# wilsonCernWq/qaray

Hardware: AMD Instinct MI355X
Metric: Msamples/s (1 sample = 1 camera path), Cornell box 1080p@512spp (higher is better)
Workload: dtype f32

## Files before the change

include/qaray_hip.h:

```cpp
#ifndef QARAY_HIP_H
#define QARAY_HIP_H

#include <stdint.h>

#include "qa_flat_scene.h"
#include "qa_photon.h"
#include "qaray_host.h"

#ifdef __cplusplus
extern "C" {
#endif

typedef struct qa_ctx qa_ctx;

typedef struct qa_counters {
  uint64_t samples;
  uint64_t casts_normal;
  uint64_t casts_shadow;
  uint64_t bvh_nodes;
  uint64_t tri_tests;
  uint64_t pixels;
} qa_counters;

#define QA_RENDER_STATS 1u
// ... 17 lines not shown
int qa_scene_edit_texels(qa_ctx *ctx, uint32_t texture, int x0, int y0, int x1, int y1, const uint8_t *rgb8, uint64_t row_stride_bytes);
int qa_scene_edit_texels_device(qa_ctx *ctx, uint32_t texture, int x0, int y0, int x1, int y1, const uint8_t *d_rgb8,
                                uint64_t row_stride_bytes, void *hip_stream);

int qa_render_region(qa_ctx *ctx, int x0, int y0, int x1, int y1, int spp_min, int spp_max,
                     int max_bounce, uint32_t seed, uint32_t flags, float *rgb, float *depth,
                     uint32_t *nsamples);
int qa_render_region_device(qa_ctx *ctx, int x0, int y0, int x1, int y1, int spp_min, int spp_max,
                            int max_bounce, uint32_t seed, uint32_t flags, float *d_rgb,
                            float *d_depth, uint32_t *d_nsamples, void *hip_stream);
#define QA_STRIP_ROWS 8
int qa_render_strips_device(qa_ctx *ctx, int x0, int y0, int x1, int y1, int first_strip, int strip_step,
                            int spp_min, int spp_max, int max_bounce, uint32_t seed, uint32_t flags,
                            float *d_rgb, float *d_depth, uint32_t *d_nsamples, void *hip_stream);
int qa_strip_count(int y0, int y1, int first_strip, int strip_step);
int qa_synchronize(qa_ctx *ctx);

int qa_photon_maps_build(qa_ctx *ctx, const qa_photon_params *params, uint32_t seed);
int qa_photon_maps_clear(qa_ctx *ctx);
int qa_photon_maps_info(qa_ctx *ctx, uint64_t emitted[2], uint64_t emissions[2]);
int qa_photon_maps_download(qa_ctx *ctx, int which, qa_photon *out, uint64_t capacity);

int qa_request_stop(qa_ctx *ctx);
int qa_clear_stop(qa_ctx *ctx);

int qa_progressive_begin(qa_ctx *ctx, int x0, int y0, int x1, int y1, int spp_min, int spp_max, int max_bounce, uint32_t seed,
                         uint32_t flags);
int qa_progressive_advance(qa_ctx *ctx, int spp_target, void *hip_stream);
int qa_progressive_read(qa_ctx *ctx, float *rgb, float *depth, uint32_t *nsamples);
int qa_progressive_read_device(qa_ctx *ctx, float *d_rgb, float *d_depth, uint32_t *d_nsamples, void *hip_stream);
// ... 200 lines not shown
```

qaray_amd/csrc/hip/qa_capi.hip:

```cpp
#include <hip/hip_runtime.h>

#include <algorithm>
#include <cstddef>
#include <cstring>
#include <new>

#include "qa_ctx.h"
#include "qa_radiance.h"
#include "qa_ray_query.h"

static int EnsurePlanSlab(qa_ctx *c)
{
  const size_t threads = (size_t) c->numCUs * 8 * QA_BLOCK;
  const bool area = c->plan.area, many = !area && c->plan.shadowLights.size() > QA_CS_LIGHT_BATCH;
  float **slab = area ? &c->dAreaSlab : many ? &c->dSurfSlab : nullptr;
  if (slab && !*slab) {
    void *p = nullptr;
    HIP_TRY(hipMalloc(&p, threads * (area ? kAreaLogFloats : 13) * sizeof(float)));
    c->sceneAllocs.push_back(p);
    c->statSceneAllocs++;
    *slab = static_cast<float *>(p);
  }
  c->ds.areaScratch = area ? c->dAreaSlab : nullptr;
  c->ds.csSurf = many ? c->dSurfSlab : nullptr;
// ... 391 lines not shown
  out->samples = h.samples;
  out->casts_normal = h.casts_normal;
  out->casts_shadow = h.casts_shadow;
  out->bvh_nodes = h.bvh_nodes;
  out->tri_tests = h.tri_tests;
  out->pixels = h.pixels;
#ifdef QA_STAMPS
  {
    const double w = (double) std::max<unsigned long long>(h.stamp[9], 1), k = (double) std::max<unsigned long long>(h.stamp[0], 1);
    fprintf(stderr, "[stamps] waves %llu, iterations/wave %.0f, cycles/wave %.3e | share of wave time: fetch+start %.3f, closest %.3f (mesh walks %.3f), shade %.3f, "
            "direct light %.3f (shadow mesh walks %.3f), sample end %.3f, miss branch %.3f, hit before shading %.3f, spawn %.3f\n", h.stamp[9], h.stamp[8] / w, k / w, h.stamp[1] / k, h.stamp[2] / k, h.stamp[3] / k,
            h.stamp[4] / k, h.stamp[5] / k, h.stamp[6] / k, h.stamp[7] / k, h.stamp[10] / k, h.stamp[11] / k, h.stamp[12] / k);
    if (h.stamp[19] || h.stamp[21])
      fprintf(stderr, "[stamps] waves without a camera ray: mesh walks of their closest-hit sweeps %.3f (the camera rays': %.3f), after the sweep %.3f | last-cast queries %.3f (mesh walks %.3f), %llu lanes asked again (of %llu casts)\n",
              h.stamp[19] / k, (h.stamp[3] - (double) h.stamp[19]) / k, h.stamp[20] / k, h.stamp[21] / k, h.stamp[22] / k, h.stamp[23], (unsigned long long) h.casts_normal);
    if (c->integ[kCs].fn && h.stamp[11])
      fprintf(stderr, "[stamps] cooperative walks: %llu rounds, %.1f of 64 lanes hold an item on average (lane occupancy of the walks %.3f); %.3f of the rounds are leaf rounds; 'mesh walks' above = the rounds alone\n", h.stamp[11],
              (double) h.stamp[10] / (double) h.stamp[11], (double) h.stamp[10] / (64.0 * (double) h.stamp[11]), (double) h.stamp[12] / (double) h.stamp[11]);
    if (c->integ[kCs].fn)
      fprintf(stderr, "[stamps] closest-hit sweeps without their rounds %.3f, winners' details %.3f, shadow sweeps without their rounds %.3f; lanes sent to the exact walks: %llu closest, %llu shadow (of %llu + %llu casts)\n",
              (h.stamp[13] - (double) h.stamp[3]) / k, h.stamp[14] / k, (h.stamp[17] - (double) h.stamp[6]) / k, h.stamp[15], h.stamp[16], (unsigned long long) h.casts_normal, (unsigned long long) h.casts_shadow);
  }
#endif
  return QA_OK;
}
int qa_reset_counters(qa_ctx *c)
{
  if (!c) return Fail(QA_EINVAL, "null context");
  if (int rc = qa_synchronize(c)) return rc;
  HIP_TRY(hipMemset(c->dCounters, 0, sizeof(DCounters)));
// ... 50 lines not shown
  return QA_OK;
}

int qa_set_option(qa_ctx *c, const char *name, long long value)
{
  if (!c || !name) return Fail(QA_EINVAL, "null argument");
  const std::string n(name);
  if (n == "coop") {
    c->optCoop = value != 0;
    if (c->haveScene) return SelectKernel(c);
  } else if (n == "cs_cull") c->optCsCull = value != 0;
  else if (n == "cs_force_exact") c->optCsForceExact = (uint32_t) (value & 3);
  else if (n == "walk_zero_terms") c->optWalkZeroTerms = value ? 1u : 0u;
  else if (n == "last_cast") c->optLastCast = value < 0 ? -1 : (value ? 1 : 0);
  else if (n == "leaf_sweep") c->optLeafSweep = value < 0 ? -1 : (value ? 1 : 0);
  else if (n == "chunk_spp") c->optChunkSpp = value < 0 ? -1 : (int) (value > 65535 ? 65535 : value);
  else if (n == "chunk_tail") c->optChunkTail = value < 0 ? 0 : (int) (value > 65535 ? 65535 : value);
  else if (n == "tile_lists") c->optTileLists = value < 0 ? -1 : (int) (value > QA_TILE_LEAF_CAP ? QA_TILE_LEAF_CAP : value);
  else if (n == "cs_pool_limit") c->optCsPool = value > 0 ? (uint32_t) std::max<long long>(64, value) : 0u;
  else if (n == "sync_samples") c->syncSamples = value < 0 ? -1 : (value > 64 ? 64 : (int) value);
  else if (n == "tile_order") c->tileOrder = value != 0;
  else if (n == "progressive_tile_limit") c->optProgTileLimit = value > 0 ? (uint32_t) std::min<long long>(value, 0x7FFFFFFF) : 0u;
  else if (n == "staged_groups") {
    c->wf.numGroups = (int) std::max<long long>(1, std::min<long long>(value, WfHost::kMaxGroups));
    if (c->haveScene) SetKernelName(c);
  } else if (n == "verbose") c->optVerbose = value != 0;
  else return Fail(QA_EINVAL, "unknown option '" + n + "'");
  return QA_OK;
}

// ... 11 lines not shown
```

qaray_amd/csrc/hip/qa_ctx.h:

```cpp
#pragma once
#include <hip/hip_runtime.h>

#include <cstdint>
#include <string>
#include <vector>

#include "qa_scene_build.h"
#include "qa_wf_types.h"
#include "qaray_hip.h"

using namespace qa;

typedef void (*KernelFn)(const DScene, const RenderParams);
KernelFn PickKernel(bool resident, bool lights, bool tex, bool area, bool stats);
KernelFn PickLastCastKernel();
KernelFn PickCs(bool lights, bool tex, bool cull, bool many, bool area);
KernelFn PickCsResume(bool lights, bool cull, bool many, bool area);
extern const int kMaxPath;
extern const size_t kAreaLogFloats;
size_t CsLdsBytes(uint32_t items, uint32_t slots);

inline thread_local std::string g_err;
inline int Fail(int code, const std::string &msg) { g_err = msg; return code; }
#define HIP_TRY(expr)                                                                          \
  do {                                                                                         \
    hipError_t e_ = (expr);                                                                    \
    if (e_ != hipSuccess) return Fail(QA_EHIP, std::string(#expr) + ": " + hipGetErrorString(e_)); \
  } while (0)

inline const char *DevEnv(const char *name)
// ... 135 lines not shown
  int syncSamples = -1;
  bool photonReady = false;
  void *dPhotons[2] = {nullptr, nullptr};
  void *dPmTables[2][3] = {{nullptr, nullptr, nullptr}, {nullptr, nullptr, nullptr}};
  void *dHeap = nullptr;
  qa_photon_params photonParams{};
  uint64_t photonEmitted[2] = {0, 0}, photonEmissions[2] = {0, 0};
  std::vector<qa_photon> hostPhotons[2];
  WfHost wf;
  std::string kernelName;
  std::string launchedName;
  bool optCoop = true;
  bool optCsCull = true;
  int optLastCast = -1;
  int optLeafSweep = -1;
  uint32_t optWalkZeroTerms = 0;
  uint32_t optCsForceExact = 0;
  uint32_t optCsPool = 0;
  bool optVerbose = false;
  uint32_t optProgTileLimit = 0;
  struct Progressive {
    bool active = false;
    bool stale = false;
    std::string ended;
    FrameArgs args;
    unsigned tiles = 0;
    size_t npix = 0;
    int target = 0;
    int top = 0;
    uint32_t *dState = nullptr;
// ... 103 lines not shown
```

qaray_amd/csrc/hip/qa_frame.hip:

```cpp
#include <algorithm>
#include <cstring>

#include "qa_ctx.h"

int EnsureHalton(qa_ctx *c, int count)
{
  if (count > c->haltonCount) {
    int n = 64;
    while (n < count) n *= 2;
    std::vector<float> t(2 * (size_t) n);
    for (int s = 0; s < n; ++s) { t[2 * s] = HaltonF(s, 11); t[2 * s + 1] = HaltonF(s, 13); }
    if (c->dHalton) (void) hipFree(c->dHalton);
    c->dHalton = nullptr;
    HIP_TRY(hipMalloc((void **) &c->dHalton, t.size() * sizeof(float)));
    HIP_TRY(hipMemcpy(c->dHalton, t.data(), t.size() * sizeof(float), hipMemcpyHostToDevice));
    c->haltonCount = n;
  }
  c->ds.halton = c->dHalton;
  c->ds.halton_count = c->haltonCount;
  return QA_OK;
}

static bool CsManyVariant(const qa_ctx *c) { return c->plan.shadowLights.size() > QA_CS_LIGHT_BATCH && !c->plan.area; }
static bool LastCastVariant(const qa_ctx *c) { return c->plan.resident && c->plan.lastCastQuery && c->ds.num_lights == 0; }
static bool CsCullVariant(const qa_ctx *c) { return c->plan.csCullOk && (CsManyVariant(c) || c->plan.area || c->plan.textured || c->ds.num_inst > 12); }

static std::string IntegratorName(const qa_ctx *c, Slot s)
{
  const ScenePlan &p = c->plan;
  const int lights = c->ds.num_lights > 0;
  char name[160];
  if (s == kCs || s == kCsResume)
    snprintf(name, sizeof(name), "qa_integrate_cs%s<LIGHTS=%d,TEX=%d,CULL=%d%s%s>", s == kCsResume ? "_resume" : "", lights, (int) p.textured, (int) CsCullVariant(c),
             CsManyVariant(c) ? ",MANY=1" : "", p.area ? ",AREA=1" : "");
  else snprintf(name, sizeof(name), "qa_integrate<RES=%d,LIGHTS=%d,TEX=%d,AREA=%d%s>", (int) p.resident, lights, (int) p.textured, (int) p.area,
                s == kMega && LastCastVariant(c) ? ",LASTCAST=1" : "");
  std::string out = name;
  if (s == kPm || s == kPmStats) out += " + photon-map gathers (PHOTON=1)";
  if (s == kMegaStats || s == kPmStats) out += " counting variant (STATS=1, reference tree)";
// ... 57 lines not shown
  return QA_OK;
}

int LaunchSetup(qa_ctx *c, Launch &L, const FrameArgs &a, int ownRows, unsigned int *work, bool resume)
{
  const hipStream_t s = a.stream;
  const int x0 = a.x0, y0 = a.y0, x1 = a.x1, y1 = a.y1;
  HIP_TRY(c->lastFrame.WaitOn(s));
  HIP_TRY(c->lastEdit.WaitOn(s));

  RenderParams &rp = L.rp;
  rp.x0 = x0; rp.y0 = y0; rp.x1 = x1; rp.y1 = y1;
  rp.spp_min = a.sppMin; rp.spp_max = a.sppMax; rp.max_bounce = a.maxBounce;
  rp.seed = a.seed;
  rp.tile_row0 = a.tileRow0; rp.tile_row_step = a.tileRowStep; rp.own_tile_rows = ownRows;
  rp.tile_lists = c->plan.tileListBytes ? (c->optTileLists < 0 ? QA_TILE_LISTS_AUTO : c->optTileLists) : 0;
  rp.sync_samples = c->syncSamples < 0 ? c->plan.syncAuto : c->syncSamples;
  rp.rgb = a.rgb; rp.depth = a.depth; rp.ns = a.ns;
  rp.work_counter = work;
  rp.tile_order = nullptr;
  {
    const int tx = (x1 - x0 + 7) / 8;
    const uint64_t key = ((uint64_t) tx << 40) ^ ((uint64_t) ownRows << 20) ^ ((uint64_t) a.tileRow0 << 8) ^ (uint64_t) a.tileRowStep ^
                         ((uint64_t) (y1 - y0) << 50);
    if (key != c->orderKey || !c->dOrder) {
      const size_t n = (size_t) tx * ownRows;
      std::vector<std::pair<float, uint32_t>> v(n);
      const float cx = 0.5f * (x1 - x0), cy = 0.5f * (y1 - y0);
      for (int r = 0; r < ownRows; ++r)
        for (int i = 0; i < tx; ++i) {
          const float px = i * 8 + 4 - cx, py = (a.tileRow0 + r * a.tileRowStep) * 8 + 4 - cy;
// ... 35 lines not shown
  if (cs && c->syncSamples < 0 && ((c->plan.syncAuto && c->plan.textured) || CsManyVariant(c))) rp.sync_samples = 32;
  if (cs && c->plan.area) rp.sync_samples = 1;
  ds.csCullOn = (c->optCsCull && c->plan.csCullOk) ? 1u : 0u;
  ds.csForceExact = c->optCsForceExact;
  ds.walkZeroTerms = c->optWalkZeroTerms;
  ds.lastCast = (LastCastVariant(c) && c->optLastCast != 0) ? (c->optLeafSweep != 0 ? 2u : 1u) : 0u;
  ds.lastCastGlow = c->plan.lastCastGlow;
  ds.csPoolLimit = DevEnv("QA_CS_POOL") ? (uint32_t) std::max(64, atoi(DevEnv("QA_CS_POOL"))) : c->optCsPool;

  L.tiles = (unsigned) ((x1 - x0 + 7) / 8) * (unsigned) ownRows;
  const long long needBlocks = ((long long) L.tiles * 64 + QA_BLOCK - 1) / QA_BLOCK;
  L.blocks = (long long) c->numCUs * (c->optBlocksPerCU > 0 ? c->optBlocksPerCU : c->integ[L.slot].blocksPerCU);
  if (pmOn && L.blocks > (long long) c->numCUs * 8) L.blocks = (long long) c->numCUs * 8;
  if (L.blocks > needBlocks) L.blocks = needBlocks;
  if (L.blocks < 1) L.blocks = 1;
  rp.chunk_spp = 0; rp.chunk_tail = 0; rp.num_chunks = 1; rp.chunk_pad = 0; rp.tile_progress = nullptr; rp.pix_state = nullptr;
  return QA_OK;
}

int LaunchFrame(qa_ctx *c, Launch &L, bool staged, hipStream_t s)
{
  EventPair ev;
  if (!c->freeEvents.empty()) { ev = c->freeEvents.back(); c->freeEvents.pop_back(); }
  else { HIP_TRY(hipEventCreate(&ev.a)); HIP_TRY(hipEventCreate(&ev.b)); }
  HIP_TRY(hipEventRecord(ev.a, s));
  if (staged) {
    const int rc = RenderStaged(c, L.ds, L.rp, s, L.rp.counters);
    if (rc != QA_OK) { c->freeEvents.push_back(ev); return rc; }
  } else {
    hipLaunchKernelGGL(c->integ[L.slot].fn, dim3((unsigned) L.blocks), dim3(QA_BLOCK), (unsigned) c->integ[L.slot].ldsBytes, s, L.ds, L.rp);
    HIP_TRY(hipGetLastError());
// ... 66 lines not shown
extern "C" {

int qa_render_region_device(qa_ctx *c, int x0, int y0, int x1, int y1, int spp_min, int spp_max, int max_bounce,
                            uint32_t seed, uint32_t flags, float *d_rgb, float *d_depth, uint32_t *d_ns, void *hip_stream)
{
  if (int rc = Enter(c)) return rc;
  return Render(c, {x0, y0, x1, y1, 0, 1, spp_min, spp_max, max_bounce, seed, flags, d_rgb, d_depth, d_ns, StreamOf(c, hip_stream)});
}

int qa_render_strips_device(qa_ctx *c, int x0, int y0, int x1, int y1, int first_strip, int strip_step, int spp_min,
                            int spp_max, int max_bounce, uint32_t seed, uint32_t flags, float *d_rgb, float *d_depth,
                            uint32_t *d_ns, void *hip_stream)
{
  if (int rc = Enter(c)) return rc;
  return Render(c, {x0, y0, x1, y1, first_strip, strip_step, spp_min, spp_max, max_bounce, seed, flags, d_rgb, d_depth, d_ns, StreamOf(c, hip_stream)});
}

int qa_strip_count(int y0, int y1, int first_strip, int strip_step)
{
  if (y1 <= y0 || first_strip < 0 || strip_step < 1) return 0;
  return OwnTileRows(y0, y1, first_strip, strip_step);
}

int qa_render_region(qa_ctx *c, int x0, int y0, int x1, int y1, int spp_min, int spp_max, int max_bounce,
                     uint32_t seed, uint32_t flags, float *rgb, float *depth, uint32_t *ns)
{
  if (!c || !rgb || !depth || !ns) return Fail(QA_EINVAL, "null argument");
  if (x1 <= x0 || y1 <= y0) return Fail(QA_EINVAL, "empty region");
  HIP_TRY(hipSetDevice(c->device));
  const size_t npix = (size_t) (x1 - x0) * (y1 - y0);
// ... 16 lines not shown
```

qaray_amd/csrc/hip/qa_kernel.h:

```cpp
#pragma once
#include <hip/hip_runtime.h>

#include <type_traits>

#include "qa_device_math.h"
#include "qa_scene_dev.h"
#include "qa_seed.h"
#include "qa_texture_dev.h"
#include "qa_tilecull.h"

namespace qa {

#ifndef QA_MIN_WAVES
#define QA_MIN_WAVES 4
#endif
#define QA_BIAS 0.005f
#define QA_DX 0.01f
#ifdef QA_WAVE_TALLIES
#define QA_TALLY(x) (x) += (unsigned long long) __popcll(__ballot(1))
#else
#define QA_LANE_TALLIES 1
#define QA_TALLY(x) (x)++
#endif

// ... 1353 lines not shown
    const uint32_t count = (uint32_t) __popcll(mask);
    if (count > limit || cursor + count > QA_TILE_LIST_CAP) continue;
    uint32_t rank = 0;
    for (unsigned long long rest = mask; rest; rest &= rest - 1) {
      const int j = __ffsll((long long) rest) - 1;
      const float bj = __shfl(bound, j);
      rank += (bj < bound || (bj == bound && j < (int) lane)) ? 1u : 0u;
    }
    if (cand) tl[QA_TILE_LIST_HDR + cursor + rank] = QA_TILE_ENTRY(word, __float_as_uint(bound));
    if (lane == 0) tl[mySlot] = 0x80000000u | (count << 8) | cursor;
    cursor += count;
  }
  __builtin_amdgcn_wave_barrier();
}

struct Path {
  Ray ray;
  f3 T;
  f3 L;
  int absorbMtl;
  int bounce;
  bool fromDiffuse;
  bool primary;
};

#define QA_MAX_PATH 8
#define QA_REC_FLOATS 19

#ifndef QA_C2_EXTRA_WAVE
#define QA_C2_EXTRA_WAVE 1
// ... 41 lines not shown
```

qaray_amd/csrc/hip/qa_kernel_lastcast_body.h:

```cpp
  extern __shared__ uint4 s_dyn[];
  SceneMem<RES> mem;
  mem.img = s_dyn;
  static_assert(RES, "the last-cast query belongs to the resident variant without lights");
  for (uint32_t i = threadIdx.x; i < sc.residentVec4; i += QA_BLOCK) s_dyn[i] = sc.resident[i];
  __syncthreads();
  uint32_t *stack = reinterpret_cast<uint32_t *>(s_dyn + sc.residentVec4) + threadIdx.x;
  float *acc = reinterpret_cast<float *>(stack + (size_t) sc.stackDepth * QA_BLOCK - threadIdx.x) + threadIdx.x;
  const uint4 *mtlTable = s_dyn + sc.resMaterials;
  for (int i = 12; i < QA_LANE_SLOTS_RES; ++i) acc[i * QA_BLOCK] = 0.f;
  constexpr bool TL = true;
  uint32_t *tileList = nullptr;
  if (rp.tile_lists > 0 && !(sc.cam.dof > 0.1f))
    tileList = reinterpret_cast<uint32_t *>(s_dyn + sc.residentVec4) + ((size_t) sc.stackDepth + QA_LANE_SLOTS_RES) * QA_BLOCK +
               __builtin_amdgcn_readfirstlane(threadIdx.x / 64) * QA_TILE_LIST_DWORDS;

  const int rw = rp.x1 - rp.x0, rh = rp.y1 - rp.y0;
  const unsigned tilesX = (unsigned) (rw + 7) / 8;
  const unsigned numTiles = tilesX * (unsigned) rp.own_tile_rows;
  const unsigned total = numTiles * (rp.chunk_spp ? rp.num_chunks : 1u) * 64u;
  const unsigned lane = __lane_id();
  unsigned curTile = 0xFFFFFFFFu, curChunk = 0;
  int chunkEnd = 0x7FFFFFFF;

  DCounters cnt = {};
// ... 3 lines not shown
  if (__lane_id() < QA_NSTAMPS) cnt.sl[__lane_id()] = 0;
#endif
  QA_T(tKernel)
  TexTables tt;
  tt.blob = sc.blob;
  tt.texels = sc.texels;
  tt.texOff = sc.texOff;
  tt.texmap = sc.texmap;
  tt.tex = sc.tex;
  tt.filter = sc.texFilter;
  RayDiff pathDiff;
  pathDiff.dx = pathDiff.dy = F3(0, 0, 1);

  uint32_t rng = 1;
  bool alive = true, needPixel = true;

  for (;;) {
    QA_T(tA)
    const unsigned long long aliveMask = __ballot(alive);
    const unsigned long long want = __ballot(alive && needPixel);
    if (want && want == aliveMask) {
      if (rp.chunk_spp && curTile != 0xFFFFFFFFu) {
        asm volatile("s_waitcnt vmcnt(0)" ::: "memory");
        if (lane == 0) __hip_atomic_store(rp.tile_progress + curTile, curChunk + 1u, __ATOMIC_RELAXED, __HIP_MEMORY_SCOPE_AGENT);
        curTile = 0xFFFFFFFFu;
      }
      unsigned base = 0;
      const int leader = __ffsll((long long) want) - 1;
      if ((int) lane == leader) base = (*rp.stop_flag) ? total : atomicAdd(rp.work_counter, 64u);
      base = __shfl(base, leader);
      unsigned item = base / 64;
      if (rp.chunk_spp && base < total) {
        curChunk = item / numTiles;
        item -= curChunk * numTiles;
        curTile = item;
        chunkEnd = (int) (rp.chunk_spp + curChunk * rp.chunk_tail);
        if (curChunk > 0) {
          for (int spins = 0; spins < (1 << 22); ++spins) {
            if (__hip_atomic_load(rp.tile_progress + curTile, __ATOMIC_RELAXED, __HIP_MEMORY_SCOPE_AGENT) >= curChunk) break;
            __builtin_amdgcn_s_sleep(16);
          }
          __builtin_amdgcn_fence(__ATOMIC_ACQUIRE, "agent");
        }
      }
      if (tileList && base < total) {
        const unsigned tile = rp.tile_order ? rp.tile_order[item] : item;
        const unsigned otr = tile / tilesX;
        buildTileLists<RES>(sc, (uint32_t) rp.tile_lists, (float) (rp.x0 + (int) ((tile % tilesX) * 8)),
                            (float) (rp.y0 + (int) (((unsigned) rp.tile_row0 + otr * (unsigned) rp.tile_row_step) * 8)), tileList,
                            reinterpret_cast<TileCone *>(stack - lane));
        rng = 1;
// ... 213 lines not shown
#undef QA_PAIR
          needPixel = true;
        }
      } else {
        rp.rgb[3 * qo + 0] = mean.x;
        rp.rgb[3 * qo + 1] = mean.y;
        rp.rgb[3 * qo + 2] = mean.z;
        rp.ns[qo] = (uint32_t) sidx;
        if (rp.chunk_spp)
          __hip_atomic_store(reinterpret_cast<unsigned long long *>(rp.pix_state) + 4 * (size_t) qo, 0x80000000ull << 32, __ATOMIC_RELAXED, __HIP_MEMORY_SCOPE_AGENT);
        QA_TALLY(cnt.pixels);
        needPixel = true;
      }
    }
    QA_TACC(cnt.sl[7], tE)
  }

  unsigned long long v[6] = {cnt.samples, cnt.casts_normal, cnt.casts_shadow, cnt.bvh_nodes, cnt.tri_tests, cnt.pixels};
  unsigned long long *dst = reinterpret_cast<unsigned long long *>(rp.counters);
  for (int i = 0; i < 6; ++i) {
    unsigned long long x = v[i];
#ifdef QA_LANE_TALLIES
    for (int off = 32; off > 0; off >>= 1) x += __shfl_down(x, off);
#endif
    if (lane == 0 && x) atomicAdd(&dst[i], x);
  }
#ifdef QA_STAMPS
  if (lane == 0) {
    cnt.sl[0] = __builtin_readcyclecounter() - tKernel;
    cnt.sl[9] = 1;
    for (int i = 0; i < QA_NSTAMPS; ++i) atomicAdd(&dst[6 + i], cnt.sl[i]);
// ... 3 lines not shown
```

qaray_amd/csrc/hip/qa_lastcast.hip:

```cpp
#include "qa_kernel.h"
#include "qa_ctx.h"

KernelFn PickLastCastKernel() { return (KernelFn) qa::qa_integrate_lastcast<true>; }
```

qaray_amd/csrc/hip/qa_probes.hip:

```cpp
#include <cstring>

#include "qa_device_math.h"
#include "qa_texture_dev.h"
#include "qa_ctx.h"

namespace qa {
__global__ __launch_bounds__(256, 8) void qa_scrub_scratch(uint32_t pattern, uint32_t *never)
{
  volatile uint32_t a[512];
  for (int i = 0; i < 512; ++i) a[i] = pattern;
  for (int i = 0; i < 300; ++i) __builtin_amdgcn_s_sleep(127);
  if (a[threadIdx.x] == 0x12345u && pattern != 0x12345u) never[0] = 1;
}
}

__global__ void qa_sincos_probe(const float *x, int n, float *s, float *c)
{
  const int i = blockIdx.x * blockDim.x + threadIdx.x;
  if (i < n) { s[i] = qsinf(x[i]); c[i] = qcosf(x[i]); }
}

__global__ void qa_math_probe(int fn, const float *x, const float *y, int n, float *out)
{
  const int i = blockIdx.x * blockDim.x + threadIdx.x;
// ... 166 lines not shown
  int mesh = 0, elem = 0;
  if (!TexProbeArgsOk(h, t.plan, op, index, n, &mesh, &elem)) return QA_EINVAL;
  TexTables tt;
  tt.blob = static_cast<const unsigned char *>(blob);
  tt.texels = reinterpret_cast<const float4 *>(t.texels.data());
  tt.texOff = t.texOff.data();
  tt.texmap = QA_BLOB_PTR(qa_texmap, blob, h->off_texmaps);
  tt.tex = QA_BLOB_PTR(qa_texture, blob, h->off_textures);
  tt.filter = t.taps.data();
  const DTri *tris = op == 8 ? t.mesh[mesh].tris.data() + elem : nullptr;
  const float *vt = op == 8 ? t.mesh[mesh].vt.data() + 6 * (size_t) elem : nullptr;
  for (int i = 0; i < n; ++i) TexProbeOne(tt, tris, vt, op, index, in + (size_t) QA_TEXPROBE_IN * i, out + (size_t) QA_TEXPROBE_OUT * i);
  return QA_OK;
}

int qa_debug_scrub_scratch(qa_ctx *c, uint32_t pattern)
{
  if (int rc = Enter(c)) return rc;
  std::vector<hipStream_t> streams = {c->stream};
  for (int g = 0; g < c->wf.numGroups; ++g) streams.push_back(c->wf.groups[g].stream);
  streams.push_back(c->wf.redoStream);
  for (hipStream_t s : streams)
    if (s) {
      hipLaunchKernelGGL(qa::qa_scrub_scratch, dim3((unsigned) c->numCUs * 8), dim3(256), 0, s, pattern, reinterpret_cast<uint32_t *>(c->dCounters));
      HIP_TRY(hipGetLastError());
    }
  HIP_TRY(hipDeviceSynchronize());
  return QA_OK;
}

// ... 2 lines not shown
```

qaray_amd/csrc/hip/qa_scene_dev.h:

```cpp
#pragma once
#include <stdint.h>

#include "qa_flat_scene.h"
#include "qa_photon.h"

#define QA_BLOCK 256
#define QA_DONE 0xFFFFFFFFu
#define QA_CS_INDEX_MASK 0xFFFFFu
#define QA_CS_LIGHT_BATCH 4
#define QA_CS_EXACT_STACK 64

namespace qa {

struct alignas(32) DNode {
  float box[6];
  uint32_t data;
  uint32_t pad;
};

struct alignas(16) DTri {
  float N[3];
  float A[3];
  float bu, bv, cu, cv;
  float s;
// ... 164 lines not shown

struct RenderParams {
  int32_t x0, y0, x1, y1;
  int32_t spp_min, spp_max, max_bounce;
  uint32_t seed;
  int32_t tile_row0, tile_row_step, own_tile_rows;
  int32_t tile_lists;
  int32_t sync_samples;
  float *rgb;
  float *depth;
  uint32_t *ns;
  const uint32_t *tile_order;
  unsigned int *work_counter;
  const volatile int *stop_flag;
  DCounters *counters;
  uint32_t chunk_spp, chunk_tail, num_chunks, chunk_pad;
  uint32_t *tile_progress;
  uint32_t *pix_state;
  DPhotonMap pm[2];
  uint2 *heap;
};

#define QA_RAYS_PER_SAMPLE 1u
#define QA_RAYS_MISS_ENVIRONMENT 2u
struct RayBatch {
  const float *o, *d;
  const float *dx, *dy;
  const float *screen;
  const uint32_t *stream;
  uint32_t n, flags;
};
// ... 3 lines not shown
```

qaray_amd/hip.py:

```python
import collections
import ctypes as C
import os

import numpy as np


_HERE = os.path.dirname(os.path.abspath(__file__))
HIP_LIB_PATH = os.environ.get("QA_HIP_LIB") or os.path.join(_HERE, "lib", "libqaray_hip.so")

QA_RENDER_STATS = 1
DEFAULT_SEED = 0x51A7A7


class Counters(C.Structure):
    _fields_ = [("samples", C.c_uint64), ("casts_normal", C.c_uint64), ("casts_shadow", C.c_uint64),
                ("bvh_nodes", C.c_uint64), ("tri_tests", C.c_uint64), ("pixels", C.c_uint64)]

    def as_dict(self):
        return {k: int(getattr(self, k)) for k, _ in self._fields_}


class PhotonMapParams(C.Structure):
    _fields_ = [("size", C.c_uint32), ("bounce", C.c_uint32), ("radius", C.c_float)]

# ... 233 lines not shown
            import torch
        except ImportError:
            pass
        L = C.CDLL(HIP_LIB_PATH)
        L.qa_last_error.restype = C.c_char_p
        L.qa_ctx_create.argtypes = [C.c_int, C.POINTER(C.c_void_p)]
        L.qa_ctx_destroy.argtypes = [C.c_void_p]
        L.qa_scene_upload.argtypes = [C.c_void_p, C.c_void_p, C.c_uint64]
        L.qa_scene_upload_device.argtypes = [C.c_void_p, C.c_void_p, C.c_uint64]
        L.qa_render_region.argtypes = [C.c_void_p] + [C.c_int] * 7 + [C.c_uint32, C.c_uint32, C.c_void_p, C.c_void_p, C.c_void_p]
        L.qa_render_region_device.argtypes = [C.c_void_p] + [C.c_int] * 7 + [C.c_uint32, C.c_uint32, C.c_void_p,
                                                                            C.c_void_p, C.c_void_p, C.c_void_p]
        L.qa_render_strips_device.argtypes = [C.c_void_p] + [C.c_int] * 9 + [C.c_uint32, C.c_uint32, C.c_void_p,
                                                                            C.c_void_p, C.c_void_p, C.c_void_p]
        L.qa_strip_count.argtypes = [C.c_int] * 4
        L.qa_synchronize.argtypes = [C.c_void_p]
        L.qa_request_stop.argtypes = [C.c_void_p]
        L.qa_clear_stop.argtypes = [C.c_void_p]
        L.qa_get_counters.argtypes = [C.c_void_p, C.POINTER(Counters)]
        L.qa_reset_counters.argtypes = [C.c_void_p]
        L.qa_get_kernel_time.argtypes = [C.c_void_p, C.POINTER(C.c_double), C.POINTER(C.c_uint64)]
        L.qa_reset_kernel_time.argtypes = [C.c_void_p]
        L.qa_set_launch_config.argtypes = [C.c_void_p, C.c_int, C.c_int]
        L.qa_debug_scrub_scratch.argtypes = [C.c_void_p, C.c_uint32]
        L.qa_set_pipeline.argtypes = [C.c_void_p, C.c_int]
        L.qa_set_option.argtypes = [C.c_void_p, C.c_char_p, C.c_longlong]
        L.qa_get_kernel_name.argtypes = [C.c_void_p]
        L.qa_get_kernel_name.restype = C.c_char_p
        L.qa_get_staged_stats.argtypes = [C.c_void_p, C.POINTER(C.c_uint64)]
        L.qa_progressive_begin.argtypes = [C.c_void_p] + [C.c_int] * 7 + [C.c_uint32, C.c_uint32]
# ... 84 lines not shown
def _check(rc):
    if rc != 0:
        raise HipError(rc, lib().qa_last_error().decode())


def tile_error_host(state):
    if not isinstance(state, np.ndarray) or state.dtype != np.uint32 or state.ndim != 3 or state.shape[2] != 8 or state.shape[0] < 1 or state.shape[1] < 1:
        raise ValueError("state: a uint32 array of shape (h, w, 8) is expected")
    state = np.ascontiguousarray(state)
    h, w = state.shape[:2]
    out = np.zeros(((h + 7) // 8, (w + 7) // 8), np.float32)
    _check(lib().qa_test_tile_error_host(state.ctypes.data, w, h, out.ctypes.data))
    return out


def tile_select_host(error, levels, target, max_tiles=0, min_error=0.0):
    error = np.ascontiguousarray(error, dtype=np.float32)
    levels = np.ascontiguousarray(levels, dtype=np.uint32)
    if error.shape != levels.shape or error.size < 1:
        raise ValueError("error and levels must have one shape and at least one tile")
    if not min_error >= 0.0:
        raise ValueError("min_error must not be negative or a NaN")
    mask = np.zeros(error.shape, np.uint8)
    v = (C.c_uint64 * 4)()
    _check(lib().qa_test_tile_select_host(error.ctypes.data, levels.ctypes.data, error.size, int(target), int(max_tiles), float(min_error),
                                          mask.ctypes.data, v))
    return mask.astype(bool), {"selected": int(v[0]), "candidates": int(v[1]), "cut_bits": int(v[2]), "max_finite_bits": int(v[3])}


def display_host(rgb, depth, ns, spp_max, srgb=True):
# ... 694 lines not shown
        self.synchronize()
        return {k: v.cpu().numpy() for k, v in out.items()}

    def render_strips_device(self, region, first_strip, strip_step, spp, rgb, depth, ns, max_bounce=5,
                             seed=DEFAULT_SEED, spp_max=None, stats=False, stream=None):
        x0, y0, x1, y1 = region
        n = strip_count(y0, y1, first_strip, strip_step) * 8 * (x1 - x0)
        assert rgb.is_cuda and rgb.is_contiguous() and rgb.numel() == 3 * n and rgb.element_size() == 4
        assert depth.is_cuda and depth.is_contiguous() and depth.numel() == n and depth.element_size() == 4
        assert ns.is_cuda and ns.is_contiguous() and ns.numel() == n and ns.element_size() == 4
        spp_max = spp if spp_max is None else spp_max
        sptr = self._stream_arg(stream, rgb)
        _check(lib().qa_render_strips_device(self._h, x0, y0, x1, y1, first_strip, strip_step, spp, spp_max,
                                             max_bounce, seed, QA_RENDER_STATS if stats else 0, rgb.data_ptr(),
                                             depth.data_ptr(), ns.data_ptr(), sptr))

    @staticmethod
    def _stream_arg(stream, tensor):
        if stream:
            return C.c_void_p(stream)
        import torch
        torch.cuda.current_stream(tensor.device).synchronize()
        return None

    def synchronize(self):
        _check(lib().qa_synchronize(self._h))

    def request_stop(self):
        _check(lib().qa_request_stop(self._h))

# ... 369 lines not shown
```

Before: 28260.

## Skip path tracing for screen tiles whose ray cone misses every instance

```diff
diff --git a/include/qaray_hip.h b/include/qaray_hip.h
--- a/include/qaray_hip.h
+++ b/include/qaray_hip.h
@@ -55,6 +55,8 @@
                             int spp_min, int spp_max, int max_bounce, uint32_t seed, uint32_t flags,
                             float *d_rgb, float *d_depth, uint32_t *d_nsamples, void *hip_stream);
 int qa_strip_count(int y0, int y1, int first_strip, int strip_step);
+int qa_empty_tiles_device(qa_ctx *ctx, int x0, int y0, int x1, int y1, int first_strip, int strip_step, uint8_t *d_mask, void *hip_stream);
+int qa_test_empty_tiles_host(const void *blob, int x0, int y0, int x1, int y1, int first_strip, int strip_step, uint8_t *mask);
 int qa_synchronize(qa_ctx *ctx);
 
 int qa_photon_maps_build(qa_ctx *ctx, const qa_photon_params *params, uint32_t seed);
diff --git a/qaray_amd/csrc/hip/qa_capi.hip b/qaray_amd/csrc/hip/qa_capi.hip
--- a/qaray_amd/csrc/hip/qa_capi.hip
+++ b/qaray_amd/csrc/hip/qa_capi.hip
@@ -429,6 +429,8 @@
     if (h.stamp[19] || h.stamp[21])
       fprintf(stderr, "[stamps] waves without a camera ray: mesh walks of their closest-hit sweeps %.3f (the camera rays': %.3f), after the sweep %.3f | last-cast queries %.3f (mesh walks %.3f), %llu lanes asked again (of %llu casts)\n",
               h.stamp[19] / k, (h.stamp[3] - (double) h.stamp[19]) / k, h.stamp[20] / k, h.stamp[21] / k, h.stamp[22] / k, h.stamp[23], (unsigned long long) h.casts_normal);
+    if (!c->integ[kCs].fn && h.stamp[16])
+      fprintf(stderr, "[stamps] turns of empty tiles: %llu of %llu turns (%.3f), share of wave time %.4f\n", h.stamp[16], h.stamp[8], (double) h.stamp[16] / (double) std::max<unsigned long long>(h.stamp[8], 1), h.stamp[15] / k);
     if (c->integ[kCs].fn && h.stamp[11])
       fprintf(stderr, "[stamps] cooperative walks: %llu rounds, %.1f of 64 lanes hold an item on average (lane occupancy of the walks %.3f); %.3f of the rounds are leaf rounds; 'mesh walks' above = the rounds alone\n", h.stamp[11],
               (double) h.stamp[10] / (double) h.stamp[11], (double) h.stamp[10] / (64.0 * (double) h.stamp[11]), (double) h.stamp[12] / (double) h.stamp[11]);
@@ -509,6 +511,7 @@
   else if (n == "walk_zero_terms") c->optWalkZeroTerms = value ? 1u : 0u;
   else if (n == "last_cast") c->optLastCast = value < 0 ? -1 : (value ? 1 : 0);
   else if (n == "leaf_sweep") c->optLeafSweep = value < 0 ? -1 : (value ? 1 : 0);
+  else if (n == "empty_tiles") c->optEmptyTiles = value < 0 ? -1 : (value ? 1 : 0);
   else if (n == "chunk_spp") c->optChunkSpp = value < 0 ? -1 : (int) (value > 65535 ? 65535 : value);
   else if (n == "chunk_tail") c->optChunkTail = value < 0 ? 0 : (int) (value > 65535 ? 65535 : value);
   else if (n == "tile_lists") c->optTileLists = value < 0 ? -1 : (int) (value > QA_TILE_LEAF_CAP ? QA_TILE_LEAF_CAP : value);
diff --git a/qaray_amd/csrc/hip/qa_ctx.h b/qaray_amd/csrc/hip/qa_ctx.h
--- a/qaray_amd/csrc/hip/qa_ctx.h
+++ b/qaray_amd/csrc/hip/qa_ctx.h
@@ -14,6 +14,7 @@
 typedef void (*KernelFn)(const DScene, const RenderParams);
 KernelFn PickKernel(bool resident, bool lights, bool tex, bool area, bool stats);
 KernelFn PickLastCastKernel();
+int LaunchEmptyTileMask(const DScene &ds, const RenderParams &rp, unsigned tiles, uint8_t *d_mask, hipStream_t s);
 KernelFn PickCs(bool lights, bool tex, bool cull, bool many, bool area);
 KernelFn PickCsResume(bool lights, bool cull, bool many, bool area);
 extern const int kMaxPath;
@@ -179,6 +180,7 @@
   bool optCsCull = true;
   int optLastCast = -1;
   int optLeafSweep = -1;
+  int optEmptyTiles = -1;
   uint32_t optWalkZeroTerms = 0;
   uint32_t optCsForceExact = 0;
   uint32_t optCsPool = 0;
diff --git a/qaray_amd/csrc/hip/qa_emptytile.h b/qaray_amd/csrc/hip/qa_emptytile.h
--- /dev/null
+++ b/qaray_amd/csrc/hip/qa_emptytile.h
@@ -0,0 +1,74 @@
+#pragma once
+#include "qa_tilecull.h"
+
+#ifndef QA_EMPTY_TILES
+#define QA_EMPTY_TILES 1
+#endif
+#define QA_EMPTY_TILE_NODES 64
+
+namespace qa {
+
+__host__ __device__ __forceinline__ float emptySpherePad(float oAbs)
+{
+  const float x = 1.2e-5f * (oAbs * oAbs + 1.f);
+  return x / (qsqrt(1.f + x) + 1.f);
+}
+
+__host__ __device__ __forceinline__ bool emptyFinite(float v) { return (v - v) == 0.f; }
+
+template <class S>
+__host__ __device__ __forceinline__ bool tileIsEmpty(const S &s, const DCamera &cam, const float *background, int numInst, bool rootIdentity,
+                                                      float X0, float Y0, TileCone *cone)
+{
+  if (numInst > QA_EMPTY_TILE_NODES) return false;
+  if (!(emptyFinite(background[0]) && emptyFinite(background[1]) && emptyFinite(background[2]))) return false;
+  TileLens lens;
+  {
+    f3 cW[4];
+    tileWindow(ld3(cam.screenA), ld3(cam.screenU), ld3(cam.screenV), X0, Y0, cW);
+    lens = tileLens(ld3(cam.pos), cW);
+  }
+  for (int k = 1; k < numInst; ++k) {
+    const int type = s.inst(k).obj_type;
+    if (type == QA_OBJ_NONE) continue;
+    const int depth = s.inst(k).depth;
+    if (depth > QA_MAX_NODE_DEPTH) return false;
+    {
+      f3 o = ld3(cam.pos), c[4];
+      tileWindow(ld3(cam.screenA), ld3(cam.screenU), ld3(cam.screenV), X0, Y0, c);
+      for (int lvl = rootIdentity ? 1 : 0; lvl <= depth; ++lvl) {
+        int a = k;
+        for (int up = depth; up > lvl; --up) a = s.inst(a).parent;
+        const qa_instance &in = s.inst(a);
+        o = tileNodePoint(in, o);
+        for (int i = 0; i < 4; ++i) c[i] = tileNodePoint(in, c[i]);
+      }
+#if defined(__HIP_DEVICE_COMPILE__)
+      __builtin_amdgcn_wave_barrier();
+#endif
+      tileCone(lens, o, c, cone);
+      if (type != QA_OBJ_MESH) cone->open = 0u;
+#if defined(__HIP_DEVICE_COMPILE__)
+      asm volatile("" ::: "memory");
+#endif
+    }
+    f3 bmin, bmax;
+    float pad = 0.f;
+    if (type == QA_OBJ_MESH) {
+      bmin = ld3(s.mesh(s.inst(k).mesh).bmin);
+      bmax = ld3(s.mesh(s.inst(k).mesh).bmax);
+    } else if (type == QA_OBJ_PLANE) {
+      bmin = F3(-1.f, -1.f, 0.f);
+      bmax = F3(1.f, 1.f, 0.f);
+    } else {
+      bmin = F3(-1.f, -1.f, -1.f);
+      bmax = F3(1.f, 1.f, 1.f);
+      pad = emptySpherePad(cone->oAbs);
+    }
+    float tLow;
+    if (tileConeMeetsBox(cone, bmin, bmax, pad, &tLow)) return false;
+  }
+  return true;
+}
+
+}
diff --git a/qaray_amd/csrc/hip/qa_frame.hip b/qaray_amd/csrc/hip/qa_frame.hip
--- a/qaray_amd/csrc/hip/qa_frame.hip
+++ b/qaray_amd/csrc/hip/qa_frame.hip
@@ -2,6 +2,7 @@
 #include <cstring>
 
 #include "qa_ctx.h"
+#include "qa_emptytile.h"
 
 int EnsureHalton(qa_ctx *c, int count)
 {
@@ -23,6 +24,11 @@
 
 static bool CsManyVariant(const qa_ctx *c) { return c->plan.shadowLights.size() > QA_CS_LIGHT_BATCH && !c->plan.area; }
 static bool LastCastVariant(const qa_ctx *c) { return c->plan.resident && c->plan.lastCastQuery && c->ds.num_lights == 0; }
+static int TileListLimit(const qa_ctx *c) { return c->plan.tileListBytes ? (c->optTileLists < 0 ? QA_TILE_LISTS_AUTO : c->optTileLists) : 0; }
+static bool EmptyTilesOn(const qa_ctx *c)
+{
+  return QA_EMPTY_TILES && LastCastVariant(c) && c->optEmptyTiles != 0 && TileListLimit(c) > 0 && !(c->ds.cam.dof > 0.1f);
+}
 static bool CsCullVariant(const qa_ctx *c) { return c->plan.csCullOk && (CsManyVariant(c) || c->plan.area || c->plan.textured || c->ds.num_inst > 12); }
 
 static std::string IntegratorName(const qa_ctx *c, Slot s)
@@ -110,7 +116,7 @@
   rp.spp_min = a.sppMin; rp.spp_max = a.sppMax; rp.max_bounce = a.maxBounce;
   rp.seed = a.seed;
   rp.tile_row0 = a.tileRow0; rp.tile_row_step = a.tileRowStep; rp.own_tile_rows = ownRows;
-  rp.tile_lists = c->plan.tileListBytes ? (c->optTileLists < 0 ? QA_TILE_LISTS_AUTO : c->optTileLists) : 0;
+  rp.tile_lists = TileListLimit(c);
   rp.sync_samples = c->syncSamples < 0 ? c->plan.syncAuto : c->syncSamples;
   rp.rgb = a.rgb; rp.depth = a.depth; rp.ns = a.ns;
   rp.work_counter = work;
@@ -176,7 +182,8 @@
   if (pmOn && L.blocks > (long long) c->numCUs * 8) L.blocks = (long long) c->numCUs * 8;
   if (L.blocks > needBlocks) L.blocks = needBlocks;
   if (L.blocks < 1) L.blocks = 1;
-  rp.chunk_spp = 0; rp.chunk_tail = 0; rp.num_chunks = 1; rp.chunk_pad = 0; rp.tile_progress = nullptr; rp.pix_state = nullptr;
+  rp.chunk_spp = 0; rp.chunk_tail = 0; rp.num_chunks = 1; rp.tile_progress = nullptr; rp.pix_state = nullptr;
+  rp.empty_tiles = (!resume && EmptyTilesOn(c)) ? 1u : 0u;
   return QA_OK;
 }
 
@@ -273,6 +280,27 @@
 {
   if (int rc = Enter(c)) return rc;
   return Render(c, {x0, y0, x1, y1, first_strip, strip_step, spp_min, spp_max, max_bounce, seed, flags, d_rgb, d_depth, d_ns, StreamOf(c, hip_stream)});
+}
+
+int qa_empty_tiles_device(qa_ctx *c, int x0, int y0, int x1, int y1, int first_strip, int strip_step, uint8_t *d_mask, void *hip_stream)
+{
+  if (int rc = Enter(c)) return rc;
+  if (!c->haveScene) return Fail(QA_ENOSCENE, "no scene uploaded");
+  if (x0 < 0 || y0 < 0 || x1 > c->ds.cam.width || y1 > c->ds.cam.height || x1 <= x0 || y1 <= y0) return Fail(QA_EINVAL, "region outside the image");
+  if (!d_mask || first_strip < 0 || strip_step < 1) return Fail(QA_EINVAL, "bad argument");
+  const int ownRows = OwnTileRows(y0, y1, first_strip, strip_step);
+  if (ownRows == 0) return QA_OK;
+  const hipStream_t s = StreamOf(c, hip_stream);
+  const unsigned tiles = (unsigned) ((x1 - x0 + 7) / 8) * (unsigned) ownRows;
+  HIP_TRY(c->lastEdit.WaitOn(s));
+  if (!EmptyTilesOn(c)) {
+    HIP_TRY(hipMemsetAsync(d_mask, 0, tiles, s));
+    return QA_OK;
+  }
+  RenderParams rp = {};
+  rp.x0 = x0; rp.y0 = y0; rp.x1 = x1; rp.y1 = y1;
+  rp.tile_row0 = first_strip; rp.tile_row_step = strip_step; rp.own_tile_rows = ownRows;
+  return LaunchEmptyTileMask(c->ds, rp, tiles, d_mask, s);
 }
 
 int qa_strip_count(int y0, int y1, int first_strip, int strip_step)
diff --git a/qaray_amd/csrc/hip/qa_kernel.h b/qaray_amd/csrc/hip/qa_kernel.h
--- a/qaray_amd/csrc/hip/qa_kernel.h
+++ b/qaray_amd/csrc/hip/qa_kernel.h
@@ -8,6 +8,7 @@
 #include "qa_seed.h"
 #include "qa_texture_dev.h"
 #include "qa_tilecull.h"
+#include "qa_emptytile.h"
 
 namespace qa {
 
@@ -1391,6 +1392,13 @@
   __builtin_amdgcn_wave_barrier();
 }
 
+template <bool RES>
+struct EmptyTileScene {
+  const DScene &sc;
+  __device__ __forceinline__ decltype(auto) inst(int k) const { return instAt<RES>(sc, k); }
+  __device__ __forceinline__ decltype(auto) mesh(int i) const { return meshAt<RES>(sc, i); }
+};
+
 struct Path {
   Ray ray;
   f3 T;
diff --git a/qaray_amd/csrc/hip/qa_kernel_lastcast_body.h b/qaray_amd/csrc/hip/qa_kernel_lastcast_body.h
--- a/qaray_amd/csrc/hip/qa_kernel_lastcast_body.h
+++ b/qaray_amd/csrc/hip/qa_kernel_lastcast_body.h
@@ -41,6 +41,19 @@
 
   uint32_t rng = 1;
   bool alive = true, needPixel = true;
+#if QA_EMPTY_TILES
+#ifdef QA_WAVE_TALLIES
+#define QA_TALLY_N(x, n) (x) += (unsigned long long) (n) * (unsigned long long) __popcll(__ballot(1))
+#else
+#define QA_TALLY_N(x, n) (x) += (unsigned long long) (n)
+#endif
+#ifdef QA_STAMPS
+  bool tileEmpty = false;
+#define QA_EMPTY_ASK true
+#else
+#define QA_EMPTY_ASK (rp.empty_tiles != 0)
+#endif
+#endif
 
   for (;;) {
     QA_T(tA)
@@ -62,6 +75,41 @@
         item -= curChunk * numTiles;
         curTile = item;
         chunkEnd = (int) (rp.chunk_spp + curChunk * rp.chunk_tail);
+#if QA_EMPTY_TILES
+      }
+      if (tileList && QA_EMPTY_ASK && base < total) {
+        const unsigned tile = rp.tile_order ? rp.tile_order[item] : item;
+        const unsigned otr = tile / tilesX;
+        const bool emptyTile = __builtin_amdgcn_readfirstlane((int) tileIsEmpty(
+            EmptyTileScene<RES>{sc}, sc.cam, sc.background, sc.num_inst, sc.rootIdentity != 0, (float) (rp.x0 + (int) ((tile % tilesX) * 8)),
+            (float) (rp.y0 + (int) (((unsigned) rp.tile_row0 + otr * (unsigned) rp.tile_row_step) * 8)), reinterpret_cast<TileCone *>(stack - lane)));
+#ifdef QA_STAMPS
+        tileEmpty = emptyTile;
+#endif
+        if (emptyTile && rp.empty_tiles) {
+          if (alive && (!rp.chunk_spp || curChunk == 0)) {
+            const unsigned tx = (tile % tilesX) * 8 + (lane % 8);
+            const unsigned ty = ((unsigned) rp.tile_row0 + otr * (unsigned) rp.tile_row_step) * 8 + (lane / 8);
+            if (tx < (unsigned) rw && ty < (unsigned) rh) {
+              const unsigned q = (otr * 8 + (lane / 8)) * (unsigned) rw + tx;
+              const f3 L0 = F3(0, 0, 0) + F3(1, 1, 1) * ld3(sc.background);
+              const f3 mean = F3(0, 0, 0) + (L0 - F3(0, 0, 0)) / 1.f;
+              rp.rgb[3 * q + 0] = mean.x;
+              rp.rgb[3 * q + 1] = mean.y;
+              rp.rgb[3 * q + 2] = mean.z;
+              rp.depth[q] = QA_BIGFLOAT;
+              rp.ns[q] = (uint32_t) rp.spp_min;
+              QA_TALLY_N(cnt.samples, rp.spp_min);
+              QA_TALLY_N(cnt.casts_normal, rp.spp_min);
+              QA_TALLY_N(cnt.pixels, 1);
+            }
+          }
+          curTile = 0xFFFFFFFFu;
+          continue;
+        }
+      }
+      if (rp.chunk_spp && base < total) {
+#endif
         if (curChunk > 0) {
           for (int spins = 0; spins < (1 << 22); ++spins) {
             if (__hip_atomic_load(rp.tile_progress + curTile, __ATOMIC_RELAXED, __HIP_MEMORY_SCOPE_AGENT) >= curChunk) break;
@@ -305,7 +353,17 @@
       }
     }
     QA_TACC(cnt.sl[7], tE)
+#if QA_EMPTY_TILES && defined(QA_STAMPS)
+    if (tileEmpty) {
+      QA_TACC(cnt.sl[15], tA)
+      if (lane == 0) cnt.sl[16] += 1;
+    }
+#endif
   }
+#if QA_EMPTY_TILES
+#undef QA_TALLY_N
+#undef QA_EMPTY_ASK
+#endif
 
   unsigned long long v[6] = {cnt.samples, cnt.casts_normal, cnt.casts_shadow, cnt.bvh_nodes, cnt.tri_tests, cnt.pixels};
   unsigned long long *dst = reinterpret_cast<unsigned long long *>(rp.counters);
diff --git a/qaray_amd/csrc/hip/qa_lastcast.hip b/qaray_amd/csrc/hip/qa_lastcast.hip
--- a/qaray_amd/csrc/hip/qa_lastcast.hip
+++ b/qaray_amd/csrc/hip/qa_lastcast.hip
@@ -2,3 +2,23 @@
 #include "qa_ctx.h"
 
 KernelFn PickLastCastKernel() { return (KernelFn) qa::qa_integrate_lastcast<true>; }
+
+namespace qa {
+__global__ __launch_bounds__(64) void qa_empty_tile_mask(const DScene sc, const RenderParams rp, unsigned tiles, uint8_t *mask)
+{
+  const unsigned tile = blockIdx.x * 64u + threadIdx.x;
+  if (tile >= tiles) return;
+  const unsigned tilesX = (unsigned) (rp.x1 - rp.x0 + 7) / 8;
+  const unsigned otr = tile / tilesX;
+  TileCone cone;
+  mask[tile] = tileIsEmpty(EmptyTileScene<true>{sc}, sc.cam, sc.background, sc.num_inst, sc.rootIdentity != 0, (float) (rp.x0 + (int) ((tile % tilesX) * 8)),
+                           (float) (rp.y0 + (int) (((unsigned) rp.tile_row0 + otr * (unsigned) rp.tile_row_step) * 8)), &cone) ? 1 : 0;
+}
+}
+
+int LaunchEmptyTileMask(const DScene &ds, const RenderParams &rp, unsigned tiles, uint8_t *d_mask, hipStream_t s)
+{
+  hipLaunchKernelGGL(qa::qa_empty_tile_mask, dim3((tiles + 63) / 64), dim3(64), 0, s, ds, rp, tiles, d_mask);
+  HIP_TRY(hipGetLastError());
+  return QA_OK;
+}
diff --git a/qaray_amd/csrc/hip/qa_probes.hip b/qaray_amd/csrc/hip/qa_probes.hip
--- a/qaray_amd/csrc/hip/qa_probes.hip
+++ b/qaray_amd/csrc/hip/qa_probes.hip
@@ -3,6 +3,7 @@
 #include "qa_device_math.h"
 #include "qa_texture_dev.h"
 #include "qa_ctx.h"
+#include "qa_emptytile.h"
 
 namespace qa {
 __global__ __launch_bounds__(256, 8) void qa_scrub_scratch(uint32_t pattern, uint32_t *never)
@@ -204,6 +205,36 @@
   return QA_OK;
 }
 
+struct EmptyTileSceneHost {
+  const qa_instance *insts;
+  const DMesh *meshes;
+  const qa_instance &inst(int k) const { return insts[k]; }
+  const DMesh &mesh(int i) const { return meshes[i]; }
+};
+
+int qa_test_empty_tiles_host(const void *blob, int x0, int y0, int x1, int y1, int first_strip, int strip_step, uint8_t *mask)
+{
+  if (!blob || !mask || first_strip < 0 || strip_step < 1) return QA_EINVAL;
+  const qa_flat_header *h = static_cast<const qa_flat_header *>(blob);
+  if (h->magic != QA_FLAT_MAGIC || h->version != QA_FLAT_VERSION) return QA_EINVAL;
+  SceneTables t;
+  std::string err;
+  const int rc = BuildScene(static_cast<const unsigned char *>(blob), h->total_bytes, BuildKnobs(), t, &err);
+  if (rc != QA_OK) return rc;
+  const DScene &ds = t.ds;
+  if (x0 < 0 || y0 < 0 || x1 > ds.cam.width || y1 > ds.cam.height || x1 <= x0 || y1 <= y0) return QA_EINVAL;
+  const int tilesX = (x1 - x0 + 7) / 8, tilesY = (y1 - y0 + 7) / 8;
+  const bool on = QA_EMPTY_TILES && t.plan.resident && t.plan.lastCastQuery && ds.num_lights == 0 && t.plan.tileListBytes && !(ds.cam.dof > 0.1f);
+  const EmptyTileSceneHost s = {QA_BLOB_PTR(qa_instance, blob, h->off_instances), t.plan.meshes.data()};
+  size_t n = 0;
+  for (int row = first_strip; row < tilesY; row += strip_step)
+    for (int tx = 0; tx < tilesX; ++tx) {
+      TileCone cone;
+      mask[n++] = on && tileIsEmpty(s, ds.cam, ds.background, ds.num_inst, ds.rootIdentity != 0, (float) (x0 + tx * 8), (float) (y0 + row * 8), &cone) ? 1 : 0;
+    }
+  return QA_OK;
+}
+
 int qa_debug_scrub_scratch(qa_ctx *c, uint32_t pattern)
 {
   if (int rc = Enter(c)) return rc;
diff --git a/qaray_amd/csrc/hip/qa_scene_dev.h b/qaray_amd/csrc/hip/qa_scene_dev.h
--- a/qaray_amd/csrc/hip/qa_scene_dev.h
+++ b/qaray_amd/csrc/hip/qa_scene_dev.h
@@ -202,7 +202,8 @@
   unsigned int *work_counter;
   const volatile int *stop_flag;
   DCounters *counters;
-  uint32_t chunk_spp, chunk_tail, num_chunks, chunk_pad;
+  uint32_t chunk_spp, chunk_tail, num_chunks;
+  uint32_t empty_tiles;
   uint32_t *tile_progress;
   uint32_t *pix_state;
   DPhotonMap pm[2];
diff --git a/qaray_amd/hip.py b/qaray_amd/hip.py
--- a/qaray_amd/hip.py
+++ b/qaray_amd/hip.py
@@ -271,6 +271,8 @@
         L.qa_render_strips_device.argtypes = [C.c_void_p] + [C.c_int] * 9 + [C.c_uint32, C.c_uint32, C.c_void_p,
                                                                             C.c_void_p, C.c_void_p, C.c_void_p]
         L.qa_strip_count.argtypes = [C.c_int] * 4
+        L.qa_empty_tiles_device.argtypes = [C.c_void_p] + [C.c_int] * 6 + [C.c_void_p, C.c_void_p]
+        L.qa_test_empty_tiles_host.argtypes = [C.c_void_p] + [C.c_int] * 6 + [C.c_void_p]
         L.qa_synchronize.argtypes = [C.c_void_p]
         L.qa_request_stop.argtypes = [C.c_void_p]
         L.qa_clear_stop.argtypes = [C.c_void_p]
@@ -385,6 +387,16 @@
     return out
 
 
+def empty_tiles_host(blob, region, first_strip=0, strip_step=1):
+    blob = np.ascontiguousarray(blob)
+    x0, y0, x1, y1 = (int(v) for v in region)
+    mask = np.zeros((strip_count(y0, y1, first_strip, strip_step), (x1 - x0 + 7) // 8), np.uint8)
+    rc = lib().qa_test_empty_tiles_host(blob.ctypes.data, x0, y0, x1, y1, int(first_strip), int(strip_step), mask.ctypes.data)
+    if rc != 0:
+        raise HipError(rc, "qa_test_empty_tiles_host: bad scene or region")
+    return mask.astype(bool)
+
+
 def tile_select_host(error, levels, target, max_tiles=0, min_error=0.0):
     error = np.ascontiguousarray(error, dtype=np.float32)
     levels = np.ascontiguousarray(levels, dtype=np.uint32)
@@ -1109,6 +1121,22 @@
         _check(lib().qa_render_strips_device(self._h, x0, y0, x1, y1, first_strip, strip_step, spp, spp_max,
                                              max_bounce, seed, QA_RENDER_STATS if stats else 0, rgb.data_ptr(),
                                              depth.data_ptr(), ns.data_ptr(), sptr))
+
+    def empty_tiles_device(self, region, mask, first_strip=0, strip_step=1, stream=None):
+        x0, y0, x1, y1 = (int(v) for v in region)
+        n = strip_count(y0, y1, first_strip, strip_step) * ((x1 - x0 + 7) // 8)
+        assert mask.is_cuda and mask.is_contiguous() and mask.numel() == n and mask.element_size() == 1
+        sptr = self._stream_arg(stream, mask)
+        _check(lib().qa_empty_tiles_device(self._h, x0, y0, x1, y1, int(first_strip), int(strip_step), mask.data_ptr(), sptr))
+
+    def empty_tiles(self, region, first_strip=0, strip_step=1):
+        import torch
+        x0, y0, x1, y1 = (int(v) for v in region)
+        shape = (strip_count(y0, y1, first_strip, strip_step), (x1 - x0 + 7) // 8)
+        mask = torch.zeros(shape, dtype=torch.uint8, device=torch.device("cuda", self.device_id))
+        self.empty_tiles_device(region, mask, first_strip, strip_step)
+        self.synchronize()
+        return mask.cpu().numpy().astype(bool)
 
     @staticmethod
     def _stream_arg(stream, tensor):
```

Measured after the change: 29640 (median of 6 runs). 1.05x the previous value.
